# zhengjingsen/LidarDetection

Measured on AMD Instinct MI355X. Metric: frames/sec (fwd+NMS) PointPillar-KITTI, higher is better.
Workload: dtype f32; 1 GPU; PointPillar-KITTI bs=16 per GPU, fp32, eval BN folded: HIP voxelize + PFN; dense 2D backbone = first layer from the pillars (sparse implicit GEMM), stride-1 3x3 layers as Winograd F(4x4,3x3) on the fp32 MFMA, strided deblocks as one fused MFMA GEMM (all this repo's HIP), the two stride-2 3x3 layers MIOpen, stride-1 deblock + 1x1 heads hipBLASLt; exact HIP top-k + decode + batched rotated NMS; clou; replicas=1

## Files before the change

include/lidar_hip.h:

```cpp
#ifndef LIDAR_HIP_H
#define LIDAR_HIP_H

#include <stddef.h>
#include <stdint.h>

#ifdef __cplusplus
extern "C" {
#endif

#define LIDAR_OK 0
#define LIDAR_ERR_ARG (-1)
#define LIDAR_ERR_LAUNCH (-2)
#define LIDAR_ERR_WORKSPACE (-3)
#define LIDAR_ERR_UNSUPPORTED (-4)

size_t lidar_voxelize_workspace_bytes(int batch, int n_max, int max_voxels);
int lidar_voxelize_workspace_init(void *ws, size_t ws_bytes, int batch, int n_max, int max_voxels, void *stream);
int lidar_voxelize(const float *points, const int *point_offsets, int batch, int n_max, int num_features,
                   const float *range6, const float *voxel_size3, const int *grid3, int max_points,
                   int max_voxels, int compact, int algo, float *voxels, int *coords, int *num_points,
                   int *voxel_offsets, void *ws, size_t ws_bytes, void *stream);
int lidar_voxelize_hostoff(const float *points, const int *point_offsets, const int *host_offsets, int batch, int n_max,
                           int num_features, const float *range6, const float *voxel_size3, const int *grid3, int max_points,
                           int max_voxels, int compact, int algo, float *voxels, int *coords, int *num_points,
// ... 166 lines not shown
                                      const float *residual, int relu, float *out_features, void *stream);
size_t lidar_spconv_packed_floats(int K, int Cin, int Cout);
int lidar_spconv_pack_weights(const float *weight, int K, int Cin, int Cout, float *packed, void *stream);
int lidar_spconv_implicit_gemm_sorted_packed(const float *in_features, const int *nbr, const int *row_mask, const int *order,
                                             int n_out, int K, int Cin, int Cout, const float *packed, const float *bias,
                                             const float *residual, int relu, float *out_features, void *stream);
int lidar_spconv_wgrad(const float *in_features, const float *grad_out, const int *nbr, int n_out, int K, int Cin, int Cout,
                       float *grad_weight, void *stream);
int lidar_spconv_wgrad_mfma_supported(int K, int Cin, int Cout);
size_t lidar_spconv_wgrad_workspace_bytes(int n_out, int K, int Cin, int Cout);
int lidar_spconv_wgrad_mfma(const float *in_features, const float *grad_out, const int *nbr, const int *order, int n_out, int K,
                            int Cin, int Cout, float *grad_weight, void *ws, size_t ws_bytes, void *stream);
size_t lidar_sparse_to_dense_workspace_bytes(int batch, int D, int H, int W);
int lidar_sparse_to_dense(const float *features, const int *indices, int n, int channels, int batch, int D, int H, int W,
                          float *out, void *ws, size_t ws_bytes, void *stream);

int lidar_bias_act_nhwc(const float *in, const float *bias, long long n_pix, int C, int relu, float *out, int out_C,
                        int out_off, void *stream);
int lidar_bias_act_upsample_nhwc(const float *in, const float *bias, int batch, int h, int w, int s, int C, int relu,
                                 float *out, int out_C, int out_off, void *stream);
int lidar_dense_gemm_bias_act(const float *A, long long M, int K, const float *W, int N, const float *bias, int relu,
                              float *D, int ldd, void *ws, size_t ws_bytes, void *stream);
int lidar_dense_gemm_export_choices(int *out7, int cap);
int lidar_dense_gemm_import_choices(const int *in7, int n);

size_t lidar_wino_packed_floats(int Cin, int Cout);
int lidar_wino_supported(int Cin, int Cout);
int lidar_wino_pack_weights(const float *w, int Cin, int Cout, float *packed, void *stream);
int lidar_wino_conv3x3_nhwc(const float *in, int B, int H, int W, int Cin, const float *packed, const float *bias, int relu, int Cout,
                            float *out, int out_C, int out_off, void *stream);
int lidar_wino_conv3x3_grouped_nhwc(const float *in, int B, int H, int W, int in_C, int group_cin, int n_groups, const float *packed,
                                    const float *bias, int relu, float *out, int out_C, int out_off, void *stream);
int lidar_wino_conv3x3_grouped_compact_nhwc(const float *in, int B, int H, int W, int in_C, int group_cin, int n_groups,
                                            const float *packed, const float *bias, int relu, const int *grp_cout, const int *grp_ooff,
                                            float *out, int out_C, int out_off, void *stream);

size_t lidar_wino43_packed_floats(int Cin, int Cout);
int lidar_wino43_supported(int Cin, int Cout);
int lidar_wino43_pack_weights(const float *w, int Cin, int Cout, float *packed, void *stream);
int lidar_wino43_conv3x3_nhwc(const float *in, int B, int H, int W, int Cin, int in_C, const float *packed, const float *bias, int relu,
                              int Cout, float *out, int out_C, int out_off, void *stream);

int lidar_wino43_wgrad_supported(int Cin, int Cout);
size_t lidar_wino43_wgrad_workspace_bytes(int B, int H, int W, int Cin, int Cout);
int lidar_wino43_wgrad_nhwc(const float *x, int x_ld, const float *g, int g_ld, int B, int H, int W, int Cin, int Cout, float *dw,
                            void *ws, size_t ws_bytes, void *stream);

size_t lidar_deconv_packed_floats(int K, int N);
int lidar_deconv_supported(int K, int s, int C_up);
int lidar_deconv_pack_weights(const float *W, int K, int N, float *packed, void *stream);
int lidar_deconv_gemm_nhwc(const float *in, int B, int h, int w, int K, const float *packed, const float *bias, int relu, int s, int C_up,
                           float *out, int out_C, int out_off, void *stream);

int lidar_anchor_scores(const float *head, long long n_loc, int row_stride, int cls_off, int anchors_per_loc, int num_class,
                        float score_thresh, float *scores, unsigned char *labels, void *stream);
int lidar_decode_topk(const float *head, int batch, long long locs_per_frame, int row_stride, int box_off, int dir_off,
                      int anchors_per_loc, int num_dir_bins, const long long *top_idx, int k, const float *anchors,
                      float dir_offset, float dir_limit_offset, float period, float *boxes, void *stream);
size_t lidar_topk_workspace_bytes(int batch, long long n);
int lidar_topk_workspace_init(void *ws, size_t ws_bytes, int batch, long long n, void *stream);
int lidar_anchor_scores_hist(const float *head, int batch, long long locs_per_frame, int row_stride, int cls_off, int anchors_per_loc,
                             int num_class, float score_thresh, float *scores, unsigned char *labels, void *ws, size_t ws_bytes,
                             void *stream);
int lidar_topk_desc(const float *scores, int batch, long long n, int k, float valid_min, float score_max, int hist_ready,
                    float *top_scores, long long *top_idx, int *counts, void *ws, size_t ws_bytes, void *stream);
int lidar_post_nms_gather(const float *boxes, const float *top_scores, const long long *top_idx, const unsigned char *labels,
                          const long long *keep, const int *num_keep, int batch, int k, long long n, int keep_stride, int post,
                          float *out_boxes, float *out_scores, long long *out_labels, int *out_num, void *stream);

size_t lidar_anchor_assign_workspace_bytes(int batch, int max_gt, int num_classes);
int lidar_anchor_assign(const float *const *anchors, const long long *counts, const long long *per_loc, const long long *out_off,
                        const float *matched, const float *unmatched, const int *remap, int num_classes, int anchor_dim,
                        long long a_total, const signed char *class_of_id, const float *gt, const float *gt_enlarged, int batch,
                        int max_gt, int gt_cols, int code_size, int sincos, int norm_by_num_examples, int *labels, float *targets,
                        float *weights, void *ws, size_t ws_bytes, void *stream);

size_t lidar_anchor_loss_workspace_bytes(int batch, const long long *counts, int num_heads);
int lidar_anchor_loss_forward(const float *const *cls, const float *const *box, const float *const *dir, const long long *counts,
                              const int *cols, const int *col_off, int num_heads, const int *labels, const float *targets,
                              const float *anchors, int anchor_dim, int batch, long long n_total, int num_class, int code_size,
                              int num_dir_bins, const float *code_weights, const float *weights, int flags, float *losses, void *ws,
                              size_t ws_bytes, void *stream);
int lidar_anchor_loss_backward(const float *const *cls, const float *const *box, const float *const *dir, const long long *counts,
                               const int *cols, const int *col_off, int num_heads, const int *labels, const float *targets,
                               const float *anchors, int anchor_dim, int batch, long long n_total, int num_class, int code_size,
                               int num_dir_bins, const float *code_weights, const float *weights, int flags,
                               const float *grad_losses, float *const *d_cls, float *const *d_box, float *const *d_dir, void *ws,
                               size_t ws_bytes, void *stream);

int lidar_sparse_to_bev_nhwc(const float *features, const int *indices, int n, int channels, int batch, int D, int H, int W,
                             float *out, void *ws, size_t ws_bytes, void *stream);

int lidar_rotate_iou_eval(const float *boxes, int n, const float *query_boxes, int k, int criterion, float *iou, void *stream);

int lidar_boxes_iou_bev_cpu(const float *boxes_a, int n_a, const float *boxes_b, int n_b, float *out);
int lidar_points_in_boxes_cpu(const float *boxes, int n_boxes, const float *pts, int n_pts, int *out);

#ifdef __cplusplus
}
#endif
#endif
```

lidardetection_amd/_lib.py:

```python
import ctypes as C
import os

_HERE = os.path.dirname(os.path.abspath(__file__))
SO_PATH = os.environ.get("LIDAR_HIP_SO") or os.path.join(_HERE, "csrc", "liblidar_hip.so")

vp, i32, f32, sz = C.c_void_p, C.c_int, C.c_float, C.c_size_t

SIGNATURES = {
    "lidar_voxelize_workspace_bytes": (sz, [i32, i32, i32]),
    "lidar_voxelize_workspace_init": (i32, [vp, sz, i32, i32, i32, vp]),
    "lidar_voxelize": (i32, [vp, vp, i32, i32, i32, vp, vp, vp, i32, i32, i32, i32, vp, vp, vp, vp, vp, sz, vp]),
    "lidar_voxelize_hostoff": (i32, [vp, vp, vp, i32, i32, i32, vp, vp, vp, i32, i32, i32, i32, vp, vp, vp, vp, vp, sz, vp]),
    "lidar_voxelize_error_flag": (i32, [vp, sz, i32, i32, i32]),
    "lidar_timer_create": (vp, []),
    "lidar_timer_destroy": (None, [vp]),
    "lidar_voxelize_time_next": (None, [vp]),
    "lidar_timer_elapsed_ms": (C.c_float, [vp]),
    "lidar_timer_parts_ms": (i32, [vp, vp]),
    "lidar_voxelize_set_error_mirror": (i32, [vp, sz, i32, i32, i32, vp, vp]),
    "lidar_pillar_vfe": (i32, [vp, vp, vp, i32, vp, i32, i32, vp, vp, vp, i32, vp, vp, i32, i32, i32, vp, vp]),
    "lidar_mean_vfe": (i32, [vp, vp, i32, i32, i32, i32, vp, vp]),
    "lidar_pillar_scatter_workspace_bytes": (sz, [i32, i32, i32]),
    "lidar_pillar_scatter": (i32, [vp, vp, i32, i32, vp, i32, i32, i32, i32, i32, vp, vp, sz, vp]),
    "lidar_pillar_scatter_update": (i32, [vp, vp, i32, i32, vp, i32, i32, i32, i32, vp, vp, vp, vp]),
# ... 44 lines not shown
    "lidar_spconv_build_hash": (i32, [vp, i32, i32, i32, i32, vp, sz, vp]),
    "lidar_spconv_subm_table": (i32, [vp, i32, i32, i32, i32, i32, i32, i32, vp, sz, vp, vp]),
    "lidar_spconv_conv_table_workspace_bytes": (sz, [i32, i32, i32, i32, i32, i32, i32]),
    "lidar_spconv_conv_outputs": (i32, [vp, i32, i32, i32, i32, i32, i32, i32, i32, i32, i32, i32, i32, i32, i32, vp, i32, vp, vp, sz, vp]),
    "lidar_spconv_conv_tables": (i32, [i32, i32, i32, i32, i32, i32, i32, i32, vp, vp, vp, sz, vp]),
    "lidar_spconv_grid_init": (i32, [vp, sz, vp]),
    "lidar_spconv_grid_rows": (i32, [vp, i32, vp, i32, i32, i32, i32, vp, i32, vp]),
    "lidar_spconv_grid_table": (i32, [vp, i32, i32, i32, i32, i32, i32, i32, i32, i32, i32, i32, i32, i32, i32, vp, i32, vp, vp]),
    "lidar_spconv_grid_table_t": (i32, [vp, i32, i32, i32, i32, i32, i32, i32, i32, i32, i32, i32, i32, i32, i32, vp, i32, vp, vp]),
    "lidar_spconv_grid_pad_rows": (i32, [vp, vp, i32, vp]),
    "lidar_spconv_transpose_table": (i32, [vp, i32, i32, i32, vp, vp]),
    "lidar_spconv_grid_outputs_workspace_bytes": (sz, [i32, i32]),
    "lidar_spconv_grid_outputs": (i32, [vp, i32, i32, i32, i32, i32, i32, i32, i32, i32, i32, i32, i32, i32, i32, vp, vp, vp, vp, sz, vp]),
    "lidar_spconv_implicit_gemm": (i32, [vp, vp, i32, i32, i32, i32, vp, vp, vp, vp]),
    "lidar_spconv_implicit_gemm_fused": (i32, [vp, vp, i32, i32, i32, i32, vp, vp, vp, i32, vp, vp]),
    "lidar_spconv_row_masks": (i32, [vp, i32, i32, vp, vp]),
    "lidar_spconv_mask_group_workspace_bytes": (sz, [i32]),
    "lidar_spconv_mask_group_init": (i32, [vp, sz, vp]),
    "lidar_spconv_mask_group": (i32, [vp, i32, i32, vp, vp, vp, sz, vp]),
    "lidar_spconv_sorted_gemm_supported": (i32, [i32, i32, i32]),
    "lidar_spconv_implicit_gemm_sorted": (i32, [vp, vp, vp, vp, i32, i32, i32, i32, vp, vp, vp, i32, vp, vp]),
    "lidar_spconv_packed_floats": (sz, [i32, i32, i32]),
    "lidar_spconv_pack_weights": (i32, [vp, i32, i32, i32, vp, vp]),
    "lidar_spconv_implicit_gemm_sorted_packed": (i32, [vp, vp, vp, vp, i32, i32, i32, i32, vp, vp, vp, i32, vp, vp]),
    "lidar_spconv_wgrad": (i32, [vp, vp, vp, i32, i32, i32, i32, vp, vp]),
    "lidar_spconv_wgrad_mfma_supported": (i32, [i32, i32, i32]),
    "lidar_spconv_wgrad_workspace_bytes": (sz, [i32, i32, i32, i32]),
    "lidar_spconv_wgrad_mfma": (i32, [vp, vp, vp, vp, i32, i32, i32, i32, vp, vp, sz, vp]),
    "lidar_sparse_to_dense_workspace_bytes": (sz, [i32, i32, i32, i32]),
    "lidar_sparse_to_dense": (i32, [vp, vp, i32, i32, i32, i32, i32, i32, vp, vp, sz, vp]),
    "lidar_sparse_to_bev_nhwc": (i32, [vp, vp, i32, i32, i32, i32, i32, i32, vp, vp, sz, vp]),
    "lidar_bias_act_nhwc": (i32, [vp, vp, C.c_longlong, i32, i32, vp, i32, i32, vp]),
    "lidar_bias_act_upsample_nhwc": (i32, [vp, vp, i32, i32, i32, i32, i32, i32, vp, i32, i32, vp]),
    "lidar_dense_gemm_bias_act": (i32, [vp, C.c_longlong, i32, vp, i32, vp, i32, vp, i32, vp, sz, vp]),
    "lidar_dense_gemm_export_choices": (i32, [vp, i32]),
    "lidar_dense_gemm_import_choices": (i32, [vp, i32]),
    "lidar_wino_packed_floats": (sz, [i32, i32]),
    "lidar_wino_supported": (i32, [i32, i32]),
    "lidar_wino_pack_weights": (i32, [vp, i32, i32, vp, vp]),
    "lidar_wino_conv3x3_nhwc": (i32, [vp, i32, i32, i32, i32, vp, vp, i32, i32, vp, i32, i32, vp]),
    "lidar_wino43_packed_floats": (sz, [i32, i32]),
    "lidar_wino43_supported": (i32, [i32, i32]),
    "lidar_wino43_pack_weights": (i32, [vp, i32, i32, vp, vp]),
    "lidar_wino43_conv3x3_nhwc": (i32, [vp, i32, i32, i32, i32, i32, vp, vp, i32, i32, vp, i32, i32, vp]),
    "lidar_wino43_wgrad_supported": (i32, [i32, i32]),
    "lidar_wino43_wgrad_workspace_bytes": (sz, [i32, i32, i32, i32, i32]),
    "lidar_wino43_wgrad_nhwc": (i32, [vp, i32, vp, i32, i32, i32, i32, i32, i32, vp, vp, sz, vp]),
    "lidar_wino_conv3x3_grouped_nhwc": (i32, [vp, i32, i32, i32, i32, i32, i32, vp, vp, i32, vp, i32, i32, vp]),
    "lidar_wino_conv3x3_grouped_compact_nhwc": (i32, [vp, i32, i32, i32, i32, i32, i32, vp, vp, i32, vp, vp, vp, i32, i32, vp]),
    "lidar_deconv_packed_floats": (sz, [i32, i32]),
    "lidar_deconv_supported": (i32, [i32, i32, i32]),
    "lidar_deconv_pack_weights": (i32, [vp, i32, i32, vp, vp]),
    "lidar_deconv_gemm_nhwc": (i32, [vp, i32, i32, i32, i32, vp, vp, i32, i32, i32, vp, i32, i32, vp]),
    "lidar_anchor_scores": (i32, [vp, C.c_longlong, i32, i32, i32, i32, f32, vp, vp, vp]),
    "lidar_decode_topk": (i32, [vp, i32, C.c_longlong, i32, i32, i32, i32, i32, vp, i32, vp, f32, f32, f32, vp, vp]),
    "lidar_topk_workspace_bytes": (sz, [i32, C.c_longlong]),
    "lidar_topk_workspace_init": (i32, [vp, sz, i32, C.c_longlong, vp]),
    "lidar_anchor_scores_hist": (i32, [vp, i32, C.c_longlong, i32, i32, i32, i32, f32, vp, vp, vp, sz, vp]),
    "lidar_topk_desc": (i32, [vp, i32, C.c_longlong, i32, f32, f32, i32, vp, vp, vp, vp, sz, vp]),
    "lidar_post_nms_gather": (i32, [vp, vp, vp, vp, vp, vp, i32, i32, C.c_longlong, i32, i32, vp, vp, vp, vp, vp]),
    "lidar_anchor_assign_workspace_bytes": (sz, [i32, i32, i32]),
    "lidar_anchor_assign": (i32, [vp, vp, vp, vp, vp, vp, vp, i32, i32, C.c_longlong, vp, vp, vp, i32, i32, i32, i32, i32, i32, vp,
                                  vp, vp, vp, sz, vp]),
    "lidar_anchor_loss_workspace_bytes": (sz, [i32, vp, i32]),
    "lidar_anchor_loss_forward": (i32, [vp, vp, vp, vp, vp, vp, i32, vp, vp, vp, i32, i32, C.c_longlong, i32, i32, i32, vp, vp, i32,
                                        vp, vp, sz, vp]),
    "lidar_anchor_loss_backward": (i32, [vp, vp, vp, vp, vp, vp, i32, vp, vp, vp, i32, i32, C.c_longlong, i32, i32, i32, vp, vp, i32,
                                         vp, vp, vp, vp, vp, sz, vp]),
    "lidar_rotate_iou_eval": (i32, [vp, i32, vp, i32, i32, vp, vp]),
    "lidar_boxes_iou_bev_cpu": (i32, [vp, i32, vp, i32, vp]),
    "lidar_points_in_boxes_cpu": (i32, [vp, i32, vp, i32, vp]),
    "lidar_voxelize_cpu_scratch_bytes": (sz, [i32]),
    "lidar_voxelize_cpu": (i32, [vp, i32, i32, vp, vp, vp, i32, i32, vp, vp, vp, vp, sz]),
}

_lib = None


class LidarHipError(RuntimeError):
    pass


def lib():
    global _lib
    if _lib is None:
        if not os.path.exists(SO_PATH):
            raise LidarHipError(
                f"{SO_PATH} is missing: build it with `python -c 'import __graft_entry__ as g; g.build()'` "
                "(hipcc --offload-arch=gfx950). There is no CPU fallback.")
        _lib = C.CDLL(SO_PATH)
        for name, (res, args) in SIGNATURES.items():
            fn = getattr(_lib, name)
            fn.restype = res
            fn.argtypes = args
    return _lib


def load_variant(path):
    if not os.path.exists(path):
        raise LidarHipError(f"{path} is missing: build it with lidardetection_amd/csrc/build.py (build_variants)")
    v = C.CDLL(path)
    for name, (res, args) in SIGNATURES.items():
        fn = getattr(v, name)
        fn.restype = res
        fn.argtypes = args
    return v
# ... 45 lines not shown
```

lidardetection_amd/bev_backbone.py:

```python
import ctypes as C
import os

import torch
import torch.nn as nn
import torch.nn.functional as F

from . import _lib, wino, workspace


def bias_act_(x, bias, relu=True, out=None, out_offset=0):
    _lib.require_cuda(bias)
    if not (x.is_cuda and x.dim() == 4 and x.is_contiguous(memory_format=torch.channels_last)):
        raise _lib.LidarHipError("bias_act_: expected a channels-last CUDA tensor")
    B, C, H, W = x.shape
    if out is None:
        out, out_offset = x, 0
    elif not (out.is_contiguous(memory_format=torch.channels_last) and out.shape[0] == B and out.shape[2:] == x.shape[2:]):
        raise _lib.LidarHipError("bias_act_: output must be channels-last with the same batch / spatial shape")
    _lib.check(_lib.lib().lidar_bias_act_nhwc(_lib.ptr(x), _lib.ptr(bias), B * H * W, C, int(bool(relu)), _lib.ptr(out),
                                              out.shape[1], int(out_offset), _lib.stream()), "lidar_bias_act_nhwc")
    return out


_LT_GEMM = [os.environ.get("LIDAR_BEV_LT_GEMM", "1") != "0"]
_SPLIT_MIN = [int(os.environ.get("LIDAR_BEV_SPLIT_MIN", "8"))]
_SPLIT = [int(os.environ.get("LIDAR_BEV_SPLIT", "2"))]
_WINO = [os.environ.get("LIDAR_BEV_WINO", "1") != "0"]
_DECONV = [os.environ.get("LIDAR_BEV_DECONV", "1") != "0"]
_SPARSE_FIRST = [os.environ.get("LIDAR_BEV_SPARSE_FIRST", "1") != "0"]


def _lt_gemm(a_ptr, M, K, w_kn, bias, relu, d_ptr, ldd, device):
    ws = workspace.get("dense_gemm", 32 << 20, device)
    st = _lib.lib().lidar_dense_gemm_bias_act(a_ptr, M, K, _lib.ptr(w_kn), w_kn.shape[1], _lib.ptr(bias), int(bool(relu)), d_ptr, ldd,
                                              _lib.ptr(ws), ws.numel(), _lib.stream())
    if st == -4:
        return False
    _lib.check(st, "lidar_dense_gemm_bias_act")
    return True


def _side_streams(device, n):
    from .spconv import conv as _sc, modules as _sm
    dev = torch.device(device)
    out = []
    for pool in (_sc._SIDE_STREAMS, _sm._RULEBOOK_STREAMS)[:n]:
        st = pool.get(dev)
        if st is None:
            st = pool[dev] = torch.cuda.Stream(dev, priority=-1)
        out.append(st)
    return out


def gemm_bias_act_into_(x, w_kn, bias, out, out_offset, relu=True):
    _lib.require_cuda(w_kn, bias)
    if not (x.is_cuda and out.is_cuda and x.dtype == torch.float32 and out.dtype == torch.float32):
        raise _lib.LidarHipError("gemm_bias_act_into_: expected float32 CUDA (ROCm) tensors")
    B, K, h, w = x.shape
    N = w_kn.shape[1]
    if (not x.is_contiguous(memory_format=torch.channels_last) or not out.is_contiguous(memory_format=torch.channels_last)
            or out.shape[0] != B or out.shape[2:] != x.shape[2:] or w_kn.shape[0] != K or bias.numel() != N
            or out_offset + N > out.shape[1] or not w_kn.is_contiguous()):
        raise _lib.LidarHipError("gemm_bias_act_into_: shapes / layouts do not match")
    return _lt_gemm(_lib.ptr(x), B * h * w, K, w_kn, bias, relu, C.c_void_p(out.data_ptr() + 4 * out_offset), out.shape[1], x.device)


def rows_gemm(a2d, w_kn, bias=None, out=None):
    if _LT_GEMM[0] and a2d.is_cuda and a2d.dtype == torch.float32 and a2d.is_contiguous() and w_kn.is_contiguous():
        if out is None:
            out = torch.empty((a2d.shape[0], w_kn.shape[1]), dtype=torch.float32, device=a2d.device)
        elif not out.is_contiguous() or out.shape != (a2d.shape[0], w_kn.shape[1]):
            raise _lib.LidarHipError("rows_gemm: out must be a contiguous (M, N) tensor")
        if _lt_gemm(_lib.ptr(a2d), a2d.shape[0], a2d.shape[1], w_kn, bias, False, _lib.ptr(out), w_kn.shape[1], a2d.device):
            return out
        _LT_GEMM[0] = False
    if out is None:
        return torch.mm(a2d, w_kn) if bias is None else torch.addmm(bias, a2d, w_kn)
    return torch.mm(a2d, w_kn, out=out) if bias is None else torch.addmm(bias, a2d, w_kn, out=out)


def deconv_supported(K, s, c_up):
    return bool(_lib.lib().lidar_deconv_supported(int(K), int(s), int(c_up)))


def deconv_pack(w_kn):
    _lib.require_cuda(w_kn)
    K, N = w_kn.shape
    L = _lib.lib()
    n = L.lidar_deconv_packed_floats(K, N)
    if n == 0:
        raise _lib.LidarHipError(f"deconv_pack: unsupported shape ({K}, {N})")
    packed = torch.empty(n, dtype=torch.float32, device=w_kn.device)
    _lib.check(L.lidar_deconv_pack_weights(_lib.ptr(w_kn.contiguous()), K, N, _lib.ptr(packed), _lib.stream()), "lidar_deconv_pack_weights")
    return packed


_DECONV_MAX_BYTES = [2 ** 31 - 1]


def deconv_fits(B, K, h, w, s, out_c):
    return B * h * w * K * 4 < _DECONV_MAX_BYTES[0] and B * h * w * s * s * out_c * 4 < _DECONV_MAX_BYTES[0]


def deconv_gemm_into_(x, packed, bias, s, out, out_offset=0, relu=True):
    _lib.require_cuda(packed, bias)
    B, K, h, w = x.shape
    c_up = bias.numel()
    if not (x.is_cuda and x.dtype == torch.float32 and x.is_contiguous(memory_format=torch.channels_last) and out.is_cuda
            and out.dtype == torch.float32 and out.is_contiguous(memory_format=torch.channels_last) and out.shape[0] == B
            and tuple(out.shape[2:]) == (s * h, s * w) and 0 <= out_offset and out_offset + c_up <= out.shape[1]
            and packed.numel() == K * s * s * c_up):
        raise _lib.LidarHipError("deconv_gemm_into_: shapes / layouts do not match")
    _lib.check(_lib.lib().lidar_deconv_gemm_nhwc(_lib.ptr(x), B, h, w, K, _lib.ptr(packed), _lib.ptr(bias), int(bool(relu)), int(s), c_up,
                                                 _lib.ptr(out), out.shape[1], int(out_offset), _lib.stream()), "lidar_deconv_gemm_nhwc")
    return out


def bias_act_upsample_(y2d, bias, batch, h, w, s, out, out_offset=0, relu=True):
    _lib.require_cuda(y2d, bias)
    C = bias.numel()
    if y2d.shape != (batch * h * w, s * s * C):
        raise _lib.LidarHipError("bias_act_upsample_: GEMM output shape does not match (batch*h*w, s*s*C)")
    if not (out.is_contiguous(memory_format=torch.channels_last) and out.shape[0] == batch
            and tuple(out.shape[2:]) == (h * s, w * s)):
        raise _lib.LidarHipError("bias_act_upsample_: output must be channels-last (batch, C_out, h*s, w*s)")
    _lib.check(_lib.lib().lidar_bias_act_upsample_nhwc(_lib.ptr(y2d), _lib.ptr(bias), batch, h, w, s, C, int(bool(relu)),
                                                       _lib.ptr(out), out.shape[1], int(out_offset), _lib.stream()),
               "lidar_bias_act_upsample_nhwc")
    return out


def collect_params(*modules):
    out = []
    for m in modules:
        out += list(m.parameters()) + list(m.buffers())
    return out


def params_key(tensors):
    return tuple((t.data_ptr(), t._version) for t in tensors)


def _fold(weight, bn, out_dim, conv_bias=None):
    scale = bn.weight.detach() / torch.sqrt(bn.running_var + bn.eps)
    shift = bn.bias.detach() - bn.running_mean * scale
    if conv_bias is not None:
        shift = shift + conv_bias.detach() * scale
    shape = [1] * weight.dim()
    shape[out_dim] = -1
    return (weight.detach() * scale.view(shape)), shift.contiguous()


class _FoldedConv(tuple):

    def __new__(cls, w, b, stride, pad, packed, dilation, groups, zero_pad):
        self = super().__new__(cls, (w, b, stride, pad, packed))
        self.dilation, self.groups, self.zero_pad = dilation, groups, zero_pad
        return self


class FoldedBEVBackbone:

    def __init__(self, blocks, deblocks, heads):
        self.sources = collect_params(blocks, deblocks, *heads)
        self.source_key = params_key(self.sources)
        self.stages = []
        for blk, de in zip(blocks, deblocks):
            convs, mods, i = [], list(blk), 0
            while i < len(mods):
                zpad = (0, 0, 0, 0)
                if isinstance(mods[i], nn.ZeroPad2d):
                    zpad, i = tuple(int(v) for v in mods[i].padding), i + 1
                conv, bn = mods[i], mods[i + 1]
                assert isinstance(conv, nn.Conv2d) and isinstance(bn, nn.BatchNorm2d) and isinstance(mods[i + 2], nn.ReLU)
                assert conv.padding_mode == "zeros" and not isinstance(conv.padding, str), "FoldedBEVBackbone: explicit zero padding only"
                w, b = _fold(conv.weight, bn, 0, conv.bias)
                pad, zp = tuple(int(v) for v in conv.padding), None
                if zpad[0] == zpad[1] >= 0 and zpad[2] == zpad[3] >= 0:
                    pad = (pad[0] + zpad[2], pad[1] + zpad[0])
                else:
                    zp = zpad
                plain = tuple(conv.dilation) == (1, 1) and conv.groups == 1 and zp is None
                packed = None
                if (_WINO[0] and w.is_cuda and plain and tuple(conv.kernel_size) == (3, 3) and tuple(conv.stride) == (1, 1)
                        and pad == (1, 1) and wino.supported(w.shape[1], w.shape[0])):
                    packed = wino.pack_auto(w)
                convs.append(_FoldedConv(w.contiguous(memory_format=torch.channels_last), b, tuple(conv.stride), pad, packed,
                                         tuple(conv.dilation), conv.groups, zp))
                i += 3
            up, bn = de[0], de[1]
            assert tuple(up.dilation) == (1, 1) and up.groups == 1 and up.padding_mode == "zeros", \
                "FoldedBEVBackbone: deblocks with dilation, groups or non-zero padding modes are not supported"
            if isinstance(up, nn.ConvTranspose2d):
                w, b = _fold(up.weight, bn, 1, up.bias)
                if tuple(up.kernel_size) == tuple(up.stride) and up.stride[0] == up.stride[1] and \
                        tuple(up.padding) == (0, 0) and tuple(up.output_padding) == (0, 0):
                    w_kn = w.permute(0, 2, 3, 1).reshape(w.shape[0], -1).contiguous()
                    upc = ("gemm", w_kn, b, up.stride[0])
                    if (_DECONV[0] and w.is_cuda and up.stride[0] > 1 and deconv_supported(w_kn.shape[0], up.stride[0], b.numel())):
                        upc = ("deconv_mfma", (deconv_pack(w_kn), w_kn), b, up.stride[0])
                else:
                    upc = ("deconv", w.contiguous(memory_format=torch.channels_last), b, (up.stride, up.padding, up.output_padding))
            else:
                w, b = _fold(up.weight, bn, 0, up.bias)
                upc = ("conv", w.contiguous(memory_format=torch.channels_last), b, (up.stride, up.padding))
            self.stages.append((convs, upc))
        self.up_channels = [s[1][2].numel() for s in self.stages]
        for h in heads:
            assert tuple(h.kernel_size) == (1, 1) and tuple(h.stride) == (1, 1)
        self.head_split = [h.weight.shape[0] for h in heads]
        if heads:
            self.head_wt = torch.cat([h.weight.detach().flatten(1) for h in heads], 0).t().contiguous()
            self.head_b = torch.cat([h.bias.detach() if h.bias is not None else h.weight.new_zeros(h.weight.shape[0])
                                     for h in heads], 0).contiguous()
        self._cats = {}
        self._streams = None
        self._first_sparse = None
        c0 = self.stages[0][0][0]
        w0, b0, st0, pad0, _ = c0
        k0 = w0.shape[2]
        if (w0.is_cuda and w0.shape[2] == w0.shape[3] and st0[0] == st0[1] and pad0[0] == pad0[1] and k0 * k0 <= 31
                and c0.dilation == (1, 1) and c0.groups == 1 and c0.zero_pad is None):
            from .spconv import ops as _sops
            if _sops.sorted_gemm_supported(k0 * k0, w0.shape[1], w0.shape[0]):
                self._first_sparse = (w0.permute(2, 3, 1, 0).reshape(k0 * k0, w0.shape[1], w0.shape[0]).contiguous(), b0, k0, int(st0[0]), int(pad0[0]))

    def first_layer_from_pillars(self, pm):
        from . import pillar_ops
        from .spconv import ops as _sops
        w9, b0, k0, st0, pad0 = self._first_sparse
        nbr, OH, OW = pillar_ops.pillar_conv_table(pm.coords, pm.B, pm.nx, pm.ny, k0, st0, pad0, pm.num_voxels_dev)
        order = _sops.mask_order(nbr)
        out = _sops.indice_conv_fused(pm.features, nbr, w9, b0, None, True, order)
        return out.view(pm.B, OH, OW, w9.shape[2]).permute(0, 3, 1, 2)

    def sparse_first_ok(self):
        return self._first_sparse is not None and _SPARSE_FIRST[0]

    def features(self, canvas, slot=0, first_done=False):
        x, cat, off = canvas, None, 0
        for si, (convs, (kind, uw, ub, ustride)) in enumerate(self.stages):
            for ci, cv in enumerate(convs):
                if first_done and si == 0 and ci == 0:
                    continue
                w, b, stride, pad, packed = cv
                if packed is not None and _WINO[0] and x.is_contiguous(memory_format=torch.channels_last):
                    x = wino.conv3x3_auto(x, packed, w.shape[0], b, True)
                    continue
                if cv.zero_pad is not None:
                    x = F.pad(x, cv.zero_pad)
                x = F.conv2d(x, w, None, stride, pad, cv.dilation, cv.groups)
                if not x.is_contiguous(memory_format=torch.channels_last):
                    x = x.contiguous(memory_format=torch.channels_last)
                bias_act_(x, b)
            B, _, h, w = x.shape
            y = None
            if kind == "deconv_mfma":
                oh, ow = h * ustride, w * ustride
                if not deconv_fits(B, x.shape[1], h, w, ustride, sum(self.up_channels)):
                    kind, uw = "gemm", uw[1]
                    y = rows_gemm(x.permute(0, 2, 3, 1).reshape(B * h * w, -1), uw)
                else:
                    uw = uw[0]
            elif kind == "gemm":
                oh, ow = h * ustride, w * ustride
                if not (ustride == 1 and _LT_GEMM[0]):
                    y = rows_gemm(x.permute(0, 2, 3, 1).reshape(B * h * w, -1), uw)
            else:
                y = F.conv_transpose2d(x, uw, None, *ustride) if kind == "deconv" else F.conv2d(x, uw, None, *ustride)
                if not y.is_contiguous(memory_format=torch.channels_last):
                    y = y.contiguous(memory_format=torch.channels_last)
                oh, ow = y.shape[2], y.shape[3]
            if cat is None:
                shape = (B, sum(self.up_channels), oh, ow)
                cat = self._cats.get(slot)
                if cat is None or cat.shape != shape or cat.device != x.device:
                    cat = self._cats[slot] = torch.empty(shape, dtype=torch.float32, device=x.device,
                                                         memory_format=torch.channels_last)
            if kind == "gemm" and y is None:
                if not gemm_bias_act_into_(x, uw, ub, cat, off):
                    _LT_GEMM[0] = False
                    y = rows_gemm(x.permute(0, 2, 3, 1).reshape(B * h * w, -1), uw)
            if kind == "deconv_mfma":
                deconv_gemm_into_(x, uw, ub, ustride, cat, off)
            elif kind == "gemm":
                if y is not None:
                    bias_act_upsample_(y, ub, B, h, w, ustride, cat, off)
            else:
                bias_act_(y, ub, out=cat, out_offset=off)
            off += ub.numel()
        return cat

    def stale(self):
        return params_key(self.sources) != self.source_key

    def merged(self, canvas):
        first_done = False
        if not torch.is_tensor(canvas):
            if self.sparse_first_ok():
                canvas, first_done = self.first_layer_from_pillars(canvas), True
            else:
                canvas = canvas.dense()
        B = canvas.shape[0]
        if 1 < _SPLIT[0] <= 2 and canvas.is_cuda and B % _SPLIT[0] == 0 and B // _SPLIT[0] >= _SPLIT_MIN[0]:
            return self._merged_split(canvas, _SPLIT[0], first_done)
        cat = self.features(canvas, first_done=first_done)
        B, C, H, W = cat.shape
        out = rows_gemm(cat.permute(0, 2, 3, 1).reshape(B * H * W, C), self.head_wt, self.head_b)
        return out.view(B, H, W, -1)

    def _merged_split(self, canvas, n, first_done=False):
        dev = canvas.device
        cur = torch.cuda.current_stream(dev)
        self._streams = _side_streams(dev, n)
        B, hb = canvas.shape[0], canvas.shape[0] // n
        out = None
        for i, st in enumerate(self._streams):
            st.wait_stream(cur)
            with torch.cuda.stream(st):
                cat = self.features(canvas[i * hb:(i + 1) * hb], slot=i + 1, first_done=first_done)
                _, C, H, W = cat.shape
                if out is None:
                    with torch.cuda.stream(cur):
                        out = torch.empty((B, H, W, self.head_wt.shape[1]), dtype=torch.float32, device=dev)
                    st.wait_stream(cur)
                out.record_stream(st)
                rows_gemm(cat.permute(0, 2, 3, 1).reshape(hb * H * W, C), self.head_wt, self.head_b, out=out[i * hb:(i + 1) * hb].view(hb * H * W, -1))
        for st in self._streams:
            cur.wait_stream(st)
        return out

    def __call__(self, canvas):
        return torch.split(self.merged(canvas), self.head_split, dim=-1)
```

lidardetection_amd/csrc/build.py:

```python
import glob
import os
import subprocess
import sys

HERE = os.path.dirname(os.path.abspath(__file__))
SO = os.path.join(HERE, "liblidar_hip.so")
HIPCC = os.environ.get("HIPCC", "/opt/rocm/bin/hipcc")
FLAGS = ["--offload-arch=gfx950", "-O3", "-fPIC", "-std=c++17", "-ffp-contract=off", "-fvisibility=hidden",
         "-Wall", "-Wno-unused-function"]
EXTRA_FLAGS = {"wino43_conv.hip": ["-mllvm", "-pragma-unroll-threshold=4000000", "-Wno-inline-asm"]}


def sources():
    return sorted(glob.glob(os.path.join(HERE, "*.hip")))


def build(force=False, verbose=False):
    srcs = sources()
    deps = srcs + glob.glob(os.path.join(HERE, "*.h")) + [os.path.abspath(__file__)]
    if not force and os.path.exists(SO) and all(os.path.getmtime(SO) >= os.path.getmtime(d) for d in deps):
        return SO
    objs = []
    procs = []
    for s in srcs:
        o = s[:-4] + ".o"
        if (not force and os.path.exists(o)
                and all(os.path.getmtime(o) >= os.path.getmtime(d) for d in [s] + deps[len(srcs):])):
            objs.append(o)
            continue
        cmd = [HIPCC, *FLAGS, *EXTRA_FLAGS.get(os.path.basename(s), []), "-c", s, "-o", o]
        if verbose:
            print(" ".join(cmd))
        procs.append((s, subprocess.Popen(cmd)))
        objs.append(o)
    for s, p in procs:
        if p.wait() != 0:
            raise RuntimeError(f"hipcc failed on {s}")
    cmd = [HIPCC, "--offload-arch=gfx950", "-shared", "-fPIC", "-o", SO, *objs]
    if verbose:
        print(" ".join(cmd))
    subprocess.check_call(cmd)
    return SO


VARIANTS = {
    "vxl_nowait": ("voxelize.hip", ["-DVXL_WAIT_TICKS=0"]),
}
AB_VARIANTS = {
    "w43_aux0": ("wino43_conv.hip", ["-DW43_STORE_AUX=0"]),
    "vxl_fill_nt": ("voxelize.hip", ["-DVXL_FILL_NT=1"]),
    "vxl_share12": ("voxelize.hip", ["-DVXL_FILL_SHARE16=12"]), "vxl_share10": ("voxelize.hip", ["-DVXL_FILL_SHARE16=10"]),
    "vxl_share8": ("voxelize.hip", ["-DVXL_FILL_SHARE16=8"]),
    "dc_nowait": ("deconv_gemm.hip", ["-DDC_PROBE=1"]),
    "sc_p1": ("sparse_conv.hip", ["-DSC_PROBE=1"]), "sc_p2": ("sparse_conv.hip", ["-DSC_PROBE=2"]), "sc_p4": ("sparse_conv.hip", ["-DSC_PROBE=4"]),
    "sc_p7": ("sparse_conv.hip", ["-DSC_PROBE=7"]),
}


def variant_path(name):
    return os.path.join(HERE, f"liblidar_hip_{name}.so")


def build_variants(force=False, verbose=False, names=None):
    build(force=False, verbose=verbose)
    outs = []
    todo = VARIANTS if names is None else {n: {**VARIANTS, **AB_VARIANTS}[n] for n in names}
    for name, (src, extra) in todo.items():
        so = variant_path(name)
        s = os.path.join(HERE, src)
        deps = [s] + glob.glob(os.path.join(HERE, "*.h")) + [os.path.abspath(__file__), SO]
        if not force and os.path.exists(so) and all(os.path.getmtime(so) >= os.path.getmtime(d) for d in deps):
            outs.append(so)
            continue
        o = os.path.join(HERE, f"{src[:-4]}.{name}.o")
        cmd = [HIPCC, *FLAGS, *EXTRA_FLAGS.get(src, []), *extra, "-c", s, "-o", o]
        if verbose:
            print(" ".join(cmd))
        subprocess.check_call(cmd)
        objs = [x[:-4] + ".o" for x in sources() if os.path.basename(x) != src] + [o]
        subprocess.check_call([HIPCC, "--offload-arch=gfx950", "-shared", "-fPIC", "-o", so, *objs])
        outs.append(so)
    return outs


if __name__ == "__main__":
    print(build(force="--force" in sys.argv, verbose=True))
    print(build_variants(force="--force" in sys.argv, verbose=True))
```

Measured before the change: 3257 frames/s.

## Add custom fp32 MFMA rows-GEMM for stride-1 deblock and 1x1 heads

Adds a HIP kernel that runs the row-major GEMM with bias and activation on the fp32 MFMA. It keeps packed weights resident in LDS, pipelines A-tile buffer loads against MFMA groups, and uses a persistent grid capped at the CU count. It replaces hipBLASLt for the stride-1 deblock and the merged 1x1 detection heads, falling back to hipBLASLt when shapes or alignment are unsupported. The aim is to cut hipBLASLt overhead and fit the tiling to small N (up to 128) and K (up to 512). The risk is that a hand-written kernel may lag a tuned library GEMM for some shapes.

```diff
diff --git a/include/lidar_hip.h b/include/lidar_hip.h
--- a/include/lidar_hip.h
+++ b/include/lidar_hip.h
@@ -242,6 +242,12 @@
 int lidar_deconv_gemm_nhwc(const float *in, int B, int h, int w, int K, const float *packed, const float *bias, int relu, int s, int C_up,
                            float *out, int out_C, int out_off, void *stream);
 
+int lidar_rows_gemm_supported(int K, int N);
+size_t lidar_rows_gemm_packed_floats(int K, int N);
+int lidar_rows_gemm_pack_weights(const float *W, int K, int N, float *packed, void *stream);
+int lidar_rows_gemm_bias_act(const float *A, long long M, int K, const float *packed, int N, const float *bias, int relu, float *D,
+                             int ldd, void *stream);
+
 int lidar_anchor_scores(const float *head, long long n_loc, int row_stride, int cls_off, int anchors_per_loc, int num_class,
                         float score_thresh, float *scores, unsigned char *labels, void *stream);
 int lidar_decode_topk(const float *head, int batch, long long locs_per_frame, int row_stride, int box_off, int dir_off,
diff --git a/lidardetection_amd/_lib.py b/lidardetection_amd/_lib.py
--- a/lidardetection_amd/_lib.py
+++ b/lidardetection_amd/_lib.py
@@ -120,6 +120,10 @@
     "lidar_deconv_supported": (i32, [i32, i32, i32]),
     "lidar_deconv_pack_weights": (i32, [vp, i32, i32, vp, vp]),
     "lidar_deconv_gemm_nhwc": (i32, [vp, i32, i32, i32, i32, vp, vp, i32, i32, i32, vp, i32, i32, vp]),
+    "lidar_rows_gemm_supported": (i32, [i32, i32]),
+    "lidar_rows_gemm_packed_floats": (sz, [i32, i32]),
+    "lidar_rows_gemm_pack_weights": (i32, [vp, i32, i32, vp, vp]),
+    "lidar_rows_gemm_bias_act": (i32, [vp, C.c_longlong, i32, vp, i32, vp, i32, vp, i32, vp]),
     "lidar_anchor_scores": (i32, [vp, C.c_longlong, i32, i32, i32, i32, f32, vp, vp, vp]),
     "lidar_decode_topk": (i32, [vp, i32, C.c_longlong, i32, i32, i32, i32, i32, vp, i32, vp, f32, f32, f32, vp, vp]),
     "lidar_topk_workspace_bytes": (sz, [i32, C.c_longlong]),
diff --git a/lidardetection_amd/bev_backbone.py b/lidardetection_amd/bev_backbone.py
--- a/lidardetection_amd/bev_backbone.py
+++ b/lidardetection_amd/bev_backbone.py
@@ -28,6 +28,7 @@
 _WINO = [os.environ.get("LIDAR_BEV_WINO", "1") != "0"]
 _DECONV = [os.environ.get("LIDAR_BEV_DECONV", "1") != "0"]
 _SPARSE_FIRST = [os.environ.get("LIDAR_BEV_SPARSE_FIRST", "1") != "0"]
+_ROWS_GEMM = [os.environ.get("LIDAR_BEV_ROWS_GEMM", "1") != "0"]
 
 
 def _lt_gemm(a_ptr, M, K, w_kn, bias, relu, d_ptr, ldd, device):
@@ -52,7 +53,34 @@
     return out
 
 
-def gemm_bias_act_into_(x, w_kn, bias, out, out_offset, relu=True):
+def rows_gemm_supported(K, N):
+    return bool(_lib.lib().lidar_rows_gemm_supported(int(K), int(N)))
+
+
+def rows_gemm_pack(w_kn):
+    K, N = w_kn.shape
+    if not (_ROWS_GEMM[0] and w_kn.is_cuda and w_kn.dtype == torch.float32 and rows_gemm_supported(K, N)):
+        return None
+    L = _lib.lib()
+    packed = torch.empty(L.lidar_rows_gemm_packed_floats(K, N), dtype=torch.float32, device=w_kn.device)
+    _lib.check(L.lidar_rows_gemm_pack_weights(_lib.ptr(w_kn.contiguous()), K, N, _lib.ptr(packed), _lib.stream()), "lidar_rows_gemm_pack_weights")
+    return packed
+
+
+def rows_gemm_mfma(a_ptr, M, K, packed, N, bias, relu, d_ptr, ldd):
+    if not _ROWS_GEMM[0] or packed is None or packed.numel() != K * ((N + 15) // 16 * 16):
+        return False
+    d_addr = d_ptr.value if isinstance(d_ptr, C.c_void_p) else int(d_ptr)
+    a_addr = a_ptr.value if isinstance(a_ptr, C.c_void_p) else int(a_ptr)
+    if (M * K * 4 >= 2 ** 31 - 1 or M * ldd * 4 >= 2 ** 31 - 1 or ldd % 4 or (d_addr or 0) % 16 or (a_addr or 0) % 16
+            or (bias is not None and bias.data_ptr() % 16)):
+        return False
+    _lib.check(_lib.lib().lidar_rows_gemm_bias_act(a_ptr, M, K, _lib.ptr(packed), N, _lib.ptr(bias), int(bool(relu)), d_ptr, ldd, _lib.stream()),
+               "lidar_rows_gemm_bias_act")
+    return True
+
+
+def gemm_bias_act_into_(x, w_kn, bias, out, out_offset, relu=True, packed=None):
     _lib.require_cuda(w_kn, bias)
     if not (x.is_cuda and out.is_cuda and x.dtype == torch.float32 and out.dtype == torch.float32):
         raise _lib.LidarHipError("gemm_bias_act_into_: expected float32 CUDA (ROCm) tensors")
@@ -62,15 +90,21 @@
             or out.shape[0] != B or out.shape[2:] != x.shape[2:] or w_kn.shape[0] != K or bias.numel() != N
             or out_offset + N > out.shape[1] or not w_kn.is_contiguous()):
         raise _lib.LidarHipError("gemm_bias_act_into_: shapes / layouts do not match")
-    return _lt_gemm(_lib.ptr(x), B * h * w, K, w_kn, bias, relu, C.c_void_p(out.data_ptr() + 4 * out_offset), out.shape[1], x.device)
-
-
-def rows_gemm(a2d, w_kn, bias=None, out=None):
+    d_ptr = C.c_void_p(out.data_ptr() + 4 * out_offset)
+    if rows_gemm_mfma(_lib.ptr(x), B * h * w, K, packed, N, bias, relu, d_ptr, out.shape[1]):
+        return True
+    return _lt_gemm(_lib.ptr(x), B * h * w, K, w_kn, bias, relu, d_ptr, out.shape[1], x.device)
+
+
+def rows_gemm(a2d, w_kn, bias=None, out=None, packed=None):
     if _LT_GEMM[0] and a2d.is_cuda and a2d.dtype == torch.float32 and a2d.is_contiguous() and w_kn.is_contiguous():
         if out is None:
             out = torch.empty((a2d.shape[0], w_kn.shape[1]), dtype=torch.float32, device=a2d.device)
         elif not out.is_contiguous() or out.shape != (a2d.shape[0], w_kn.shape[1]):
             raise _lib.LidarHipError("rows_gemm: out must be a contiguous (M, N) tensor")
+        if a2d.shape[0] > 0 and rows_gemm_mfma(_lib.ptr(a2d), a2d.shape[0], a2d.shape[1], packed, w_kn.shape[1], bias, False, _lib.ptr(out),
+                                               w_kn.shape[1]):
+            return out
         if _lt_gemm(_lib.ptr(a2d), a2d.shape[0], a2d.shape[1], w_kn, bias, False, _lib.ptr(out), w_kn.shape[1], a2d.device):
             return out
         _LT_GEMM[0] = False
@@ -165,6 +199,7 @@
         self.sources = collect_params(blocks, deblocks, *heads)
         self.source_key = params_key(self.sources)
         self.stages = []
+        self.up1_packed = {}
         for blk, de in zip(blocks, deblocks):
             convs, mods, i = [], list(blk), 0
             while i < len(mods):
@@ -197,6 +232,8 @@
                         tuple(up.padding) == (0, 0) and tuple(up.output_padding) == (0, 0):
                     w_kn = w.permute(0, 2, 3, 1).reshape(w.shape[0], -1).contiguous()
                     upc = ("gemm", w_kn, b, up.stride[0])
+                    if up.stride[0] == 1:
+                        self.up1_packed[len(self.stages)] = rows_gemm_pack(w_kn)
                     if (_DECONV[0] and w.is_cuda and up.stride[0] > 1 and deconv_supported(w_kn.shape[0], up.stride[0], b.numel())):
                         upc = ("deconv_mfma", (deconv_pack(w_kn), w_kn), b, up.stride[0])
                 else:
@@ -209,10 +246,12 @@
         for h in heads:
             assert tuple(h.kernel_size) == (1, 1) and tuple(h.stride) == (1, 1)
         self.head_split = [h.weight.shape[0] for h in heads]
+        self.head_packed = None
         if heads:
             self.head_wt = torch.cat([h.weight.detach().flatten(1) for h in heads], 0).t().contiguous()
             self.head_b = torch.cat([h.bias.detach() if h.bias is not None else h.weight.new_zeros(h.weight.shape[0])
                                      for h in heads], 0).contiguous()
+            self.head_packed = rows_gemm_pack(self.head_wt)
         self._cats = {}
         self._streams = None
         self._first_sparse = None
@@ -278,7 +317,7 @@
                     cat = self._cats[slot] = torch.empty(shape, dtype=torch.float32, device=x.device,
                                                          memory_format=torch.channels_last)
             if kind == "gemm" and y is None:
-                if not gemm_bias_act_into_(x, uw, ub, cat, off):
+                if not gemm_bias_act_into_(x, uw, ub, cat, off, packed=self.up1_packed.get(si)):
                     _LT_GEMM[0] = False
                     y = rows_gemm(x.permute(0, 2, 3, 1).reshape(B * h * w, -1), uw)
             if kind == "deconv_mfma":
@@ -306,7 +345,7 @@
             return self._merged_split(canvas, _SPLIT[0], first_done)
         cat = self.features(canvas, first_done=first_done)
         B, C, H, W = cat.shape
-        out = rows_gemm(cat.permute(0, 2, 3, 1).reshape(B * H * W, C), self.head_wt, self.head_b)
+        out = rows_gemm(cat.permute(0, 2, 3, 1).reshape(B * H * W, C), self.head_wt, self.head_b, packed=self.head_packed)
         return out.view(B, H, W, -1)
 
     def _merged_split(self, canvas, n, first_done=False):
@@ -325,7 +364,8 @@
                         out = torch.empty((B, H, W, self.head_wt.shape[1]), dtype=torch.float32, device=dev)
                     st.wait_stream(cur)
                 out.record_stream(st)
-                rows_gemm(cat.permute(0, 2, 3, 1).reshape(hb * H * W, C), self.head_wt, self.head_b, out=out[i * hb:(i + 1) * hb].view(hb * H * W, -1))
+                rows_gemm(cat.permute(0, 2, 3, 1).reshape(hb * H * W, C), self.head_wt, self.head_b, out=out[i * hb:(i + 1) * hb].view(hb * H * W, -1),
+                          packed=self.head_packed)
         for st in self._streams:
             cur.wait_stream(st)
         return out
diff --git a/lidardetection_amd/csrc/build.py b/lidardetection_amd/csrc/build.py
--- a/lidardetection_amd/csrc/build.py
+++ b/lidardetection_amd/csrc/build.py
@@ -52,6 +52,8 @@
     "vxl_share12": ("voxelize.hip", ["-DVXL_FILL_SHARE16=12"]), "vxl_share10": ("voxelize.hip", ["-DVXL_FILL_SHARE16=10"]),
     "vxl_share8": ("voxelize.hip", ["-DVXL_FILL_SHARE16=8"]),
     "dc_nowait": ("deconv_gemm.hip", ["-DDC_PROBE=1"]),
+    "rg_p1": ("rows_gemm.hip", ["-DRG_PROBE=1"]), "rg_p2": ("rows_gemm.hip", ["-DRG_PROBE=2"]), "rg_p4": ("rows_gemm.hip", ["-DRG_PROBE=4"]),
+    "rg_p5": ("rows_gemm.hip", ["-DRG_PROBE=5"]),
     "sc_p1": ("sparse_conv.hip", ["-DSC_PROBE=1"]), "sc_p2": ("sparse_conv.hip", ["-DSC_PROBE=2"]), "sc_p4": ("sparse_conv.hip", ["-DSC_PROBE=4"]),
     "sc_p7": ("sparse_conv.hip", ["-DSC_PROBE=7"]),
 }
diff --git a/lidardetection_amd/csrc/rows_gemm.hip b/lidardetection_amd/csrc/rows_gemm.hip
--- /dev/null
+++ b/lidardetection_amd/csrc/rows_gemm.hip
@@ -0,0 +1,234 @@
+#include "common.h"
+#ifndef RG_PROBE
+#define RG_PROBE 0
+#endif
+
+typedef float f32x4 __attribute__((ext_vector_type(4)));
+typedef unsigned u32x4 __attribute__((ext_vector_type(4)));
+
+#define RG_OOB 0x80000000u
+#define RG_LDS_BYTES (160 * 1024)
+#define RG_ROWS 4
+
+__global__ __launch_bounds__(256) void rg_pack_kernel(const float *__restrict__ W, int K, int N, int NT, float *__restrict__ P) {
+    const long long idx = (long long)blockIdx.x * 256 + threadIdx.x;
+    if (idx >= (long long)K * NT * 16) return;
+    const int s = (int)(idx & 3), l = (int)((idx >> 2) & 63);
+    const long long jt = idx >> 8;
+    const int j = (int)(jt / NT), t = (int)(jt - (long long)j * NT);
+    const int k = 16 * j + 4 * (l >> 4) + s, col = 16 * t + (l & 15);
+    P[idx] = col < N ? W[(size_t)k * N + col] : 0.f;
+}
+
+struct RgArgs {
+    const float *A;
+    const float *pk;
+    const float *bias;
+    float *D;
+    int M, K, ldd, relu;
+    int ncols;
+    int nt_total, t0;
+    int T16;
+    unsigned a_bytes, d_bytes;
+};
+
+template <int NT, bool FIRST>
+__device__ __forceinline__ void rg_group(f32x4 (&acc)[RG_ROWS][NT], const f32x4 (&bw)[NT], const f32x4 *ap) {
+#pragma unroll
+    for (int i = 0; i < RG_ROWS; ++i) {
+#pragma unroll
+        for (int s = 0; s < 4; ++s) {
+#pragma unroll
+            for (int tt = 0; tt < NT; ++tt) {
+                if (FIRST && s == 0) {
+                    const f32x4 z = {0.f, 0.f, 0.f, 0.f};
+                    acc[i][tt] = __builtin_amdgcn_mfma_f32_16x16x4f32(bw[tt][s], ap[i][s], z, 0, 0, 0);
+                } else {
+                    acc[i][tt] = __builtin_amdgcn_mfma_f32_16x16x4f32(bw[tt][s], ap[i][s], acc[i][tt], 0, 0, 0);
+                }
+            }
+        }
+    }
+}
+
+template <int NT>
+__global__ __launch_bounds__(256) void rg_kernel(const RgArgs a) {
+    extern __shared__ float4 s_w4[];
+    const f32x4 *s_w = reinterpret_cast<const f32x4 *>(s_w4);
+    const int t = threadIdx.x, l = t & 63, wv = __builtin_amdgcn_readfirstlane(t >> 6);
+    const int K = a.K, ng = K >> 4;
+    {
+        const float4 *src = reinterpret_cast<const float4 *>(a.pk);
+        const int total = ng * NT * 64;
+        for (int idx = t; idx < total; idx += 256) {
+            const int jt = idx >> 6, j = jt / NT, tt = jt - j * NT;
+            s_w4[idx] = src[((size_t)(j * a.nt_total + a.t0 + tt) << 6) + (idx & 63)];
+        }
+    }
+    __syncthreads();
+    const int nw = (int)gridDim.x * 4, w = (int)blockIdx.x * 4 + wv;
+    const int rt_begin = (int)((long long)a.T16 * w / nw), rt_end = (int)((long long)a.T16 * (w + 1) / nw);
+    if (rt_begin >= rt_end) return;
+
+    const __amdgpu_buffer_rsrc_t arsrc = __builtin_amdgcn_make_buffer_rsrc(const_cast<float *>(a.A), (short)0, (int)a.a_bytes, 0x00020000);
+    const __amdgpu_buffer_rsrc_t drsrc = __builtin_amdgcn_make_buffer_rsrc(a.D, (short)0, (int)a.d_bytes, 0x00020000);
+    const __amdgpu_buffer_rsrc_t brsrc =
+        __builtin_amdgcn_make_buffer_rsrc(const_cast<float *>(a.bias), (short)0, a.bias ? a.ncols * 4 : 0, 0x00020000);
+    const unsigned lane_a = (unsigned)(l & 15) * (unsigned)K * 4u + (unsigned)(l >> 4) * 16u;
+    const unsigned lane_d = (unsigned)(l & 15) * (unsigned)a.ldd * 4u + (unsigned)(l >> 4) * 16u;
+    const unsigned lane_d_last = (16 * (NT - 1) + 4 * (l >> 4) < a.ncols) ? lane_d + (unsigned)(NT - 1) * 64u : RG_OOB;
+
+    auto load_pair = [&](f32x4(&buf)[2 * RG_ROWS], int rt0, int nrt, int p) {
+#pragma unroll
+        for (int h = 0; h < 2; ++h) {
+#pragma unroll
+            for (int i = 0; i < RG_ROWS; ++i) {
+                const int g = 2 * p + h;
+                unsigned sp = (i < nrt && g < ng) ? (unsigned)(rt0 + i) * (unsigned)K * 64u + (unsigned)g * 64u : RG_OOB;
+                if (RG_PROBE & 1) sp = RG_OOB;
+                buf[RG_ROWS * h + i] = __builtin_bit_cast(f32x4, __builtin_amdgcn_raw_buffer_load_b128(arsrc, (int)(lane_a + sp), 0, 0));
+            }
+        }
+    };
+    bool b_live = true;
+    auto read_b = [&](f32x4(&buf)[NT], int j) {
+        if ((RG_PROBE & 2) && !b_live) return;
+        const f32x4 *p = s_w + ((j < ng ? j : 0) * NT) * 64 + l;
+#pragma unroll
+        for (int tt = 0; tt < NT; ++tt) buf[tt] = p[tt * 64];
+    };
+
+    f32x4 acc[RG_ROWS][NT];
+    f32x4 ax[2 * RG_ROWS], ay[2 * RG_ROWS], b0[NT], b1[NT];
+    const int np2 = (ng + 3) >> 2;
+    int rt0 = rt_begin, nrt = min(RG_ROWS, rt_end - rt0);
+    load_pair(ax, rt0, nrt, 0);
+    read_b(b0, 0);
+    b_live = false;
+    for (;;) {
+        const int rt0n = rt0 + RG_ROWS;
+        const bool has_next = rt0n < rt_end;
+        const int nrtn = has_next ? min(RG_ROWS, rt_end - rt0n) : 0;
+        for (int q = 0; q < np2; ++q) {
+            const bool last_q = q + 1 == np2;
+            load_pair(ay, rt0, nrt, 2 * q + 1);
+            read_b(b1, 4 * q + 1);
+            __builtin_amdgcn_sched_barrier(0);
+            if (q == 0) rg_group<NT, true>(acc, b0, ax);
+            else rg_group<NT, false>(acc, b0, ax);
+            __builtin_amdgcn_sched_barrier(0);
+            read_b(b0, 4 * q + 2);
+            __builtin_amdgcn_sched_barrier(0);
+            if (4 * q + 1 < ng) rg_group<NT, false>(acc, b1, ax + RG_ROWS);
+            __builtin_amdgcn_sched_barrier(0);
+            if (!last_q) load_pair(ax, rt0, nrt, 2 * q + 2);
+            else load_pair(ax, rt0n, nrtn, 0);
+            read_b(b1, 4 * q + 3);
+            __builtin_amdgcn_sched_barrier(0);
+            if (4 * q + 2 < ng) rg_group<NT, false>(acc, b0, ay);
+            __builtin_amdgcn_sched_barrier(0);
+            read_b(b0, last_q ? 0 : 4 * q + 4);
+            __builtin_amdgcn_sched_barrier(0);
+            if (4 * q + 3 < ng) rg_group<NT, false>(acc, b1, ay + RG_ROWS);
+            __builtin_amdgcn_sched_barrier(0);
+        }
+        {
+            const float lo = a.relu ? 0.f : -__builtin_inff();
+            f32x4 bv[NT];
+#pragma unroll
+            for (int tt = 0; tt < NT; ++tt)
+                bv[tt] = __builtin_bit_cast(f32x4, __builtin_amdgcn_raw_buffer_load_b128(brsrc, (16 * tt + 4 * (l >> 4)) * 4, 0, 0));
+#pragma unroll
+            for (int i = 0; i < RG_ROWS; ++i) {
+                const unsigned rowb = (unsigned)(rt0 + i) * (unsigned)a.ldd * 64u;
+#pragma unroll
+                for (int tt = 0; tt < NT; ++tt) {
+                    f32x4 v = acc[i][tt] + bv[tt];
+#pragma unroll
+                    for (int r = 0; r < 4; ++r) v[r] = fmaxf(v[r], lo);
+                    const unsigned off = i < nrt ? (tt == NT - 1 ? lane_d_last : lane_d + (unsigned)tt * 64u) + rowb : RG_OOB;
+                    if (!(RG_PROBE & 4)) __builtin_amdgcn_raw_buffer_store_b128(__builtin_bit_cast(u32x4, v), drsrc, (int)off, 0, 0);
+                }
+            }
+        }
+        if (!has_next) break;
+        rt0 = rt0n;
+        nrt = nrtn;
+    }
+}
+
+LIDAR_EXPORT int lidar_rows_gemm_supported(int K, int N) { return K >= 64 && K <= 512 && (K & 15) == 0 && N >= 4 && N <= 128 && (N & 3) == 0; }
+
+LIDAR_EXPORT size_t lidar_rows_gemm_packed_floats(int K, int N) {
+    return lidar_rows_gemm_supported(K, N) ? (size_t)K * (size_t)(((N + 15) >> 4) << 4) : 0;
+}
+
+LIDAR_EXPORT int lidar_rows_gemm_pack_weights(const float *W, int K, int N, float *packed, void *stream) {
+    if (!W || !packed || !lidar_rows_gemm_supported(K, N) || (reinterpret_cast<uintptr_t>(packed) & 15)) return LIDAR_ERR_ARG;
+    const int NT = (N + 15) >> 4;
+    hipLaunchKernelGGL(rg_pack_kernel, dim3(divup((long long)K * NT * 16, 256)), dim3(256), 0, (hipStream_t)stream, W, K, N, NT, packed);
+    return lidar_check_launch("lidar_rows_gemm_pack_weights");
+}
+
+static int rg_cu_count() {
+    static int cus[64] = {};
+    int dev = 0, n = 0;
+    if (hipGetDevice(&dev) != hipSuccess) return 256;
+    dev &= 63;
+    if (cus[dev] == 0) cus[dev] = (hipDeviceGetAttribute(&n, hipDeviceAttributeMultiprocessorCount, dev) == hipSuccess && n > 0) ? n : 256;
+    return cus[dev];
+}
+
+template <int NT>
+static void rg_launch(const RgArgs &a, unsigned grid, size_t lds, hipStream_t stream) {
+    static bool attr_set[64] = {};
+    int dev_id = 0;
+    (void)hipGetDevice(&dev_id);
+    dev_id &= 63;
+    if (!attr_set[dev_id]) {
+        (void)hipFuncSetAttribute(reinterpret_cast<const void *>(&rg_kernel<NT>), hipFuncAttributeMaxDynamicSharedMemorySize, RG_LDS_BYTES);
+        attr_set[dev_id] = true;
+    }
+    hipLaunchKernelGGL(rg_kernel<NT>, dim3(grid), dim3(256), lds, stream, a);
+}
+
+LIDAR_EXPORT int lidar_rows_gemm_bias_act(const float *A, long long M, int K, const float *packed, int N, const float *bias, int relu,
+                                          float *D, int ldd, void *stream) {
+    if (!A || !packed || !D || M <= 0 || !lidar_rows_gemm_supported(K, N) || ldd < N) return LIDAR_ERR_ARG;
+    if ((reinterpret_cast<uintptr_t>(A) & 15) || (reinterpret_cast<uintptr_t>(packed) & 15) || (reinterpret_cast<uintptr_t>(D) & 15) ||
+        (reinterpret_cast<uintptr_t>(bias) & 15) || (ldd & 3) || M * K * 4 >= 0x7fffffffll || M * ldd * 4 >= 0x7fffffffll)
+        return LIDAR_ERR_ARG;
+    const int nt_total = (N + 15) >> 4;
+    int nt_max = RG_LDS_BYTES / (K * 64);
+    if (nt_max > 8) nt_max = 8;
+    const int n_slices = (nt_total + nt_max - 1) / nt_max, nt_slice = (nt_total + n_slices - 1) / n_slices;
+    RgArgs a;
+    a.A = A; a.pk = packed; a.M = (int)M; a.K = K; a.ldd = ldd; a.relu = relu; a.nt_total = nt_total;
+    a.T16 = (int)((M + 15) >> 4);
+    a.a_bytes = (unsigned)(M * K * 4);
+    long long grid = (a.T16 + 4 * RG_ROWS - 1) / (4 * RG_ROWS);
+    const long long cap = rg_cu_count();
+    if (grid > cap) grid = cap;
+    for (int t0 = 0; t0 < nt_total; t0 += nt_slice) {
+        const int nt = nt_total - t0 < nt_slice ? nt_total - t0 : nt_slice;
+        a.t0 = t0;
+        a.ncols = N - 16 * t0 < 16 * nt ? N - 16 * t0 : 16 * nt;
+        a.bias = bias ? bias + 16 * t0 : nullptr;
+        a.D = D + 16 * t0;
+        a.d_bytes = (unsigned)(((M - 1) * ldd + a.ncols) * 4);
+        const size_t lds = (size_t)K * nt * 64;
+        switch (nt) {
+        case 1: rg_launch<1>(a, (unsigned)grid, lds, (hipStream_t)stream); break;
+        case 2: rg_launch<2>(a, (unsigned)grid, lds, (hipStream_t)stream); break;
+        case 3: rg_launch<3>(a, (unsigned)grid, lds, (hipStream_t)stream); break;
+        case 4: rg_launch<4>(a, (unsigned)grid, lds, (hipStream_t)stream); break;
+        case 5: rg_launch<5>(a, (unsigned)grid, lds, (hipStream_t)stream); break;
+        case 6: rg_launch<6>(a, (unsigned)grid, lds, (hipStream_t)stream); break;
+        case 7: rg_launch<7>(a, (unsigned)grid, lds, (hipStream_t)stream); break;
+        default: rg_launch<8>(a, (unsigned)grid, lds, (hipStream_t)stream); break;
+        }
+        const int st = lidar_check_launch("lidar_rows_gemm_bias_act");
+        if (st != LIDAR_OK) return st;
+    }
+    return LIDAR_OK;
+}
```

Result: no change. 3228 frames/s (-0.9%).
